# mgholamikn/PoseGen

Measured on AMD Instinct MI355X. Metric: rendered rays/sec (512x512, 64 samples/ray), higher is better.
Workload: dtype bf16

## Files before the change

posegen_amd/csrc/pg_device.h:

```cpp
#pragma once
#include <hip/hip_runtime.h>

#include <atomic>

#include "pg_program.h"

namespace pgd {
using namespace pgl;

typedef __attribute__((ext_vector_type(8))) __bf16 bf16x8;
typedef __attribute__((ext_vector_type(8))) _Float16 f16x8;
typedef __attribute__((ext_vector_type(16))) float f32x16;

struct EvalArgs {
    const float* rays;
    const float* z;
    const float* pts;
    const float* pnoise;
    const float* skts;
    const float* cams;
    const float* codes;
    const uint8_t* wstream;
    const uint8_t* wy;
    const float* rec_ab;
// ... 15 lines not shown
    int walk_rho;
};

struct RecArgs {
    const float* rays;
    const float* skts;
    const float* cams;
    const float* codes;
    const uint8_t* wy;
    float* rec_ab;
    uint8_t* rec_y;
    const float* z;
    long long pose_stride;
    int n_rays;
    int n_codes;
    int S;
};

struct PassWalk {
    int S, G, rho, pts;
    int dq[2], dr[2];
    int it, c;
    long long p0;
    int r0, off0;
    int itn, cn, r0n, off0n;
    long long p0n;
    static __host__ __device__ __forceinline__ int uni(int v) {
#if defined(__HIP_DEVICE_COMPILE__)
        return __builtin_amdgcn_readfirstlane(v);
#else
        return v;
#endif
    }
    __host__ __device__ __forceinline__ PassWalk(int S_, int pts_, int b, int G_, int rho_) : S(S_), G(G_), rho(rho_), pts(pts_) {
        const long long s0 = (long long)pts * (G + rho), s1 = (long long)pts * rho;
        dq[0] = uni((int)(s0 / S)); dr[0] = uni((int)(s0 % S));
        dq[1] = uni((int)(s1 / S)); dr[1] = uni((int)(s1 % S));
        it = c = b;
        p0 = (long long)b * pts;
        r0 = uni((int)(p0 / S));
        off0 = uni((int)(p0 - (long long)r0 * S));
        peek();
    }
    __host__ __device__ __forceinline__ void peek() {
        const int wrap = c + rho >= G ? 1 : 0;
        const int di = wrap ? rho : G + rho;
        itn = it + di;
        cn = c + rho - (wrap ? G : 0);
        p0n = p0 + (long long)di * pts;
        off0n = off0 + dr[wrap];
        r0n = r0 + dq[wrap];
        if (off0n >= S) { off0n -= S; ++r0n; }
    }
    __host__ __device__ __forceinline__ void advance() { it = itn; c = cn; p0 = p0n; r0 = r0n; off0 = off0n; }
};

template <const int (&P)[24]>
__device__ __forceinline__ int perm_dev(int s) {
    constexpr unsigned long long lo = [] { unsigned long long v = 0; for (int i = 0; i < 12; ++i) v |= (unsigned long long)P[i] << (5 * i); return v; }();
    constexpr unsigned long long hi = [] { unsigned long long v = 0; for (int i = 0; i < 12; ++i) v |= (unsigned long long)P[12 + i] << (5 * i); return v; }();
    return (int)(((s < 12 ? lo : hi) >> (5 * (s < 12 ? s : s - 12))) & 31);
}
__device__ __forceinline__ int slot_joint_dev(int s) { return perm_dev<PERM16>(s); }

inline hipError_t ensure_lds_attr(const void* fn, int bytes, std::atomic<unsigned long long>& done) {
    int dev = 0;
    hipError_t e = hipGetDevice(&dev);
    if (e != hipSuccess) return e;
    const unsigned long long bit = 1ull << (dev & 63);
    if (done.load(std::memory_order_acquire) & bit) return hipSuccess;
    e = hipFuncSetAttribute(fn, hipFuncAttributeMaxDynamicSharedMemorySize, bytes);
    if (e != hipSuccess) return e;
    done.fetch_or(bit, std::memory_order_release);
    return hipSuccess;
}

__device__ __forceinline__ void glds16(const void* g, void* l) {
    __builtin_amdgcn_global_load_lds((const __attribute__((address_space(1))) void*)g,
                                     (__attribute__((address_space(3))) void*)l, 16, 0, 0);
}

#ifndef PG_RING_SLOTS
#define PG_RING_SLOTS 3
#endif
#ifndef PG_DMA_BASE
#define PG_DMA_BASE 0
#endif
template <int NWAVE, int NCHUNK_, int NDMA = NWAVE, int MASK_NX = 0, int MASK_X0 = 0, int MASK_X1 = 0, int MASK_X2 = -1, bool AHEAD_ = false>
struct Stream {
    static constexpr bool AHEAD = AHEAD_;
    static constexpr int NSLOT = PG_RING_SLOTS;
    static constexpr int DEPTH = NSLOT - 1;
    static constexpr int PER = CHUNK_BYTES / 1024 / NDMA;
    const uint8_t* wstream;
    uint8_t* ring;
    int wave, lane;
    uint32_t next_off;
    uint32_t fill_slot;
    uint32_t rd_off;
    uint32_t ring_lds;
    uint32_t lane16;
    uint32_t pf_mask = 0u, nx_mask = 0u;

    __device__ __forceinline__ void skip_masked() {
        if constexpr (MASK_NX > 0) {
            const uint32_t c = next_off / CHUNK_BYTES;
            const uint32_t k0 = c - (uint32_t)MASK_X0, k1 = c - (uint32_t)MASK_X1, k2 = c - (uint32_t)MASK_X2;
            const uint32_t k = k0 < (uint32_t)MASK_NX ? k0 : (MASK_X2 >= 0 && k2 < (uint32_t)MASK_NX ? k2 : k1);
            if (k < (uint32_t)MASK_NX) next_off += (uint32_t)__builtin_ctz(~(pf_mask >> k)) * CHUNK_BYTES;
        }
    }
    __device__ __forceinline__ void advance() {
        next_off = next_off + CHUNK_BYTES == (uint32_t)NCHUNK_ * CHUNK_BYTES ? 0u : next_off + CHUNK_BYTES;
        if constexpr (MASK_NX > 0) {
            if (next_off == 0u) pf_mask = nx_mask;
            skip_masked();
        }
    }

    __device__ __forceinline__ bool dma_wave() const { return NDMA == NWAVE || (wave >= dma_base() && wave < dma_base() + NDMA); }
    static constexpr int dma_base() { return NDMA == NWAVE ? 0 : PG_DMA_BASE; }
    __device__ __forceinline__ void prefetch_next() {
        const uint8_t* src = wstream + next_off + ((wave - dma_base()) * (PER * 1024) + lane * 16);
        uint8_t* dst = ring + fill_slot * CHUNK_BYTES + (wave - dma_base()) * (PER * 1024);
        if (dma_wave()) {
#pragma unroll
            for (int i = 0; i < PER; ++i) glds16(src + i * 1024, dst + i * 1024);
        }
        advance();
        fill_slot = fill_slot + 1 == NSLOT ? 0u : fill_slot + 1;
        asm volatile("" : "+s"(next_off), "+s"(fill_slot));
    }
    __device__ __forceinline__ void start(uint32_t first_mask = 0u) {
        next_off = 0;
        fill_slot = 0;
        pf_mask = nx_mask = first_mask;
        skip_masked();
#pragma unroll
        for (int i = 0; i < DEPTH; ++i) prefetch_next();
        rd_off = (uint32_t)(NSLOT - 1) * CHUNK_BYTES + lane * 16;
    }
#if defined(PG_STAMPS)
    unsigned long long t_vm = 0, t_bar = 0;
    unsigned long long t_rel = 0, t_rst = 0, t_s0 = 0, t_s1 = 0;
    unsigned n_rst = 0;
    template <bool PRIMED = false>
    __device__ __forceinline__ void restart_stamp() {
        unsigned long long t;
        asm volatile("s_memtime %0\n\ts_waitcnt lgkmcnt(0)" : "=s"(t), "+s"(t_s0), "+s"(t_s1), "+s"(t_rel)::"memory");
        if (PRIMED) { t_vm += t_s1 - t_s0; t_bar += t_rel - t_s1; }
        t_rst += t - t_rel;
        n_rst += 1u;
    }
#endif
    __device__ __forceinline__ void enter(int ) {
#if defined(PG_STAMPS)
        unsigned long long s0, s1, s2;
        asm volatile("s_waitcnt lgkmcnt(0)\n\ts_memtime %0\n\ts_waitcnt lgkmcnt(0)" : "=s"(s0)::"memory");
        asm volatile("s_waitcnt vmcnt(%0)" ::"n"((DEPTH - 1) * PER) : "memory");
        asm volatile("s_memtime %0\n\ts_waitcnt lgkmcnt(0)" : "=s"(s1)::"memory");
        __builtin_amdgcn_s_barrier();
        asm volatile("s_memtime %0\n\ts_waitcnt lgkmcnt(0)" : "=s"(s2)::"memory");
        t_vm += s1 - s0;
        t_bar += s2 - s1;
#else
        asm volatile("s_waitcnt vmcnt(%0)" ::"n"((DEPTH - 1) * PER) : "memory");
        asm volatile("s_waitcnt lgkmcnt(0)" ::: "memory");
        __builtin_amdgcn_s_barrier();
#endif
        prefetch_next();
        rd_off = rd_off + CHUNK_BYTES >= (uint32_t)NSLOT * CHUNK_BYTES + lane * 16 ? rd_off - (NSLOT - 1) * CHUNK_BYTES
                                                                                  : rd_off + CHUNK_BYTES;
        asm volatile("" : "+v"(rd_off)::"memory");
    }
    uint32_t cur_src, cur_dst;
    static constexpr bool plain_ok(int c) {
        if (c < 0) return false;
        const int n = c + DEPTH + 1;
        if (n >= NCHUNK_) return false;
        if (MASK_NX > 0) {
            const int xs[3] = {MASK_X0, MASK_X1, MASK_X2};
            for (int i = 0; i < 3; ++i)
                if (xs[i] >= 0 && c + 1 <= xs[i] + MASK_NX - 1 && n >= xs[i]) return false;
        }
        return true;
    }
    static constexpr int WAIT_NEXT = 1, PRIMED = 2;
    __device__ __forceinline__ void wait_pieces(int fl) {
        if (AHEAD && (fl & WAIT_NEXT)) asm volatile("s_waitcnt vmcnt(0)" ::: "memory");
        else asm volatile("s_waitcnt vmcnt(%0)" ::"n"((DEPTH - 1) * PER) : "memory");
    }
    __device__ __forceinline__ void ring_step(bool plain) {
        cur_src = next_off + (wave - dma_base()) * (PER * 1024);
        cur_dst = fill_slot * CHUNK_BYTES + (wave - dma_base()) * (PER * 1024);
        if (plain) next_off += CHUNK_BYTES; else advance();
        fill_slot = fill_slot + 1 == NSLOT ? 0u : fill_slot + 1;
        asm volatile("" : "+s"(next_off), "+s"(fill_slot), "+s"(cur_src), "+s"(cur_dst));
        rd_off = rd_off + CHUNK_BYTES >= (uint32_t)NSLOT * CHUNK_BYTES + lane * 16 ? rd_off - (NSLOT - 1) * CHUNK_BYTES
                                                                                  : rd_off + CHUNK_BYTES;
        asm volatile("" : "+v"(rd_off)::"memory");
    }
    __device__ __forceinline__ void enter_split(bool plain = false, int fl = 0) {
        static_assert(!AHEAD || NDMA == NWAVE, "chunk entries of the A pipe that runs across them: every wave refills");
#if defined(PG_STAMPS)
        if (AHEAD && (fl & PRIMED)) {
            ring_step(plain);
            if (fl & WAIT_NEXT)
                asm volatile("s_memtime %0\n\ts_waitcnt vmcnt(0)\n\ts_memtime %1\n\ts_barrier\n\ts_memtime %2" : "=&s"(t_s0), "=&s"(t_s1), "=&s"(t_rel)::"memory");
            else
                asm volatile("s_memtime %0\n\ts_waitcnt vmcnt(%3)\n\ts_memtime %1\n\ts_barrier\n\ts_memtime %2" : "=&s"(t_s0), "=&s"(t_s1), "=&s"(t_rel) : "n"((DEPTH - 1) * PER) : "memory");
            return;
        }
        {
            unsigned long long s0, s1, s2;
            asm volatile("s_waitcnt lgkmcnt(0)\n\ts_memtime %0\n\ts_waitcnt lgkmcnt(0)" : "=s"(s0)::"memory");
            wait_pieces(fl);
            asm volatile("s_memtime %0\n\ts_waitcnt lgkmcnt(0)" : "=s"(s1)::"memory");
            __builtin_amdgcn_s_barrier();
            asm volatile("s_memtime %0\n\ts_waitcnt lgkmcnt(0)" : "=s"(s2)::"memory");
            t_vm += s1 - s0;
            t_bar += s2 - s1;
            t_rel = s2;
        }
#else
        if (dma_wave()) wait_pieces(fl);
        if (!(AHEAD && (fl & PRIMED))) asm volatile("s_waitcnt lgkmcnt(0)" ::: "memory");
#if !defined(PG_ABL_NOBARRIER)
        __builtin_amdgcn_s_barrier();
#endif
#endif
        ring_step(plain);
    }
    __device__ __forceinline__ void piece(int i) const {
#if defined(PG_ABL_NODMA)
        return;
#endif
        if (!dma_wave()) return;
#if defined(PG_VISIBLE_DMA)
        glds16(wstream + (cur_src + i * 1024) + lane16, ring + cur_dst + i * 1024);
        return;
#endif
        const uint8_t* sbase = wstream + (cur_src + i * 1024);
        asm volatile("s_mov_b32 m0, %0\n\ts_nop 0\n\tglobal_load_lds_dwordx4 %1, %2"
                     :: "s"(ring_lds + cur_dst + i * 1024), "v"(lane16), "s"(sbase) : "memory");
    }
    __device__ __forceinline__ const uint8_t* at(int , int byte_off) const {
        return ring + byte_off + rd_off;
    }
    template <typename R>
    __device__ __forceinline__ void issue(R& dst, int pos) const {
        const unsigned addr = ring_lds + rd_off;
        switch (pos) {
#define PG_ISSUE_CASE(P) case P: asm volatile("ds_read_b128 %0, %1 offset:" #P "*1024" : "=v"(dst) : "v"(addr)); break;
            PG_ISSUE_CASE(0) PG_ISSUE_CASE(1) PG_ISSUE_CASE(2) PG_ISSUE_CASE(3) PG_ISSUE_CASE(4) PG_ISSUE_CASE(5)
            PG_ISSUE_CASE(6) PG_ISSUE_CASE(7) PG_ISSUE_CASE(8) PG_ISSUE_CASE(9) PG_ISSUE_CASE(10) PG_ISSUE_CASE(11)
            PG_ISSUE_CASE(12) PG_ISSUE_CASE(13) PG_ISSUE_CASE(14) PG_ISSUE_CASE(15) PG_ISSUE_CASE(16) PG_ISSUE_CASE(17)
            PG_ISSUE_CASE(18) PG_ISSUE_CASE(19) PG_ISSUE_CASE(20) PG_ISSUE_CASE(21) PG_ISSUE_CASE(22) PG_ISSUE_CASE(23)
            PG_ISSUE_CASE(24) PG_ISSUE_CASE(25) PG_ISSUE_CASE(26) PG_ISSUE_CASE(27) PG_ISSUE_CASE(28) PG_ISSUE_CASE(29)
            PG_ISSUE_CASE(30) PG_ISSUE_CASE(31)
#undef PG_ISSUE_CASE
            default: __builtin_unreachable();
        }
    }
    template <typename R>
    __device__ __forceinline__ void issue_next(R& dst, int pos) const {
        const unsigned addr = ring_lds + rd_off + (fill_slot == (uint32_t)(NSLOT - 1) ? 0u - (uint32_t)((NSLOT - 1) * CHUNK_BYTES) : (uint32_t)CHUNK_BYTES);
        switch (pos) {
#define PG_ISSUE_CASE(P) case P: asm volatile("ds_read_b128 %0, %1 offset:" #P "*1024" : "=v"(dst) : "v"(addr)); break;
            PG_ISSUE_CASE(0) PG_ISSUE_CASE(1) PG_ISSUE_CASE(2) PG_ISSUE_CASE(3)
#undef PG_ISSUE_CASE
            default: __builtin_unreachable();
        }
    }
    __device__ __forceinline__ void drain() const { asm volatile("s_waitcnt vmcnt(0)" ::: "memory"); }
};

__device__ __forceinline__ f32x16 load_bias(const float* bias, int tile, int h) {
    const float4* p = reinterpret_cast<const float4*>(bias + (tile * 2 + h) * 16);
    const float4 a = p[0], b = p[1], c = p[2], d = p[3];
    f32x16 r = {a.x, a.y, a.z, a.w, b.x, b.y, b.z, b.w, c.x, c.y, c.z, c.w, d.x, d.y, d.z, d.w};
    return r;
}

__device__ __forceinline__ void lds_barrier() {
    asm volatile("s_waitcnt lgkmcnt(0)" ::: "memory");
    __builtin_amdgcn_s_barrier();
    asm volatile("" ::: "memory");
}

constexpr int LDS_RING = 0;
constexpr int LDS_BIAS = PG_RING_SLOTS * CHUNK_BYTES;
constexpr int LDS_CUT = LDS_BIAS + BIAS_FLOATS * 4;
constexpr int LDS_RTAB = LDS_CUT + 48 * 4;
constexpr int LDS_TOTAL = LDS_RTAB + MAXR * SLOT_FLOATS * 4;
static_assert(LDS_BIAS % 16 == 0 && LDS_CUT % 16 == 0 && LDS_RTAB % 16 == 0, "LDS alignment");
#if !defined(PG_RING_EXPERIMENT)
static_assert(LDS_TOTAL <= 160 * 1024, "LDS budget of one CU");
#endif

__device__ __forceinline__ void bone_local(const float* sk, float px, float py, float pz,
                                           float& qx, float& qy, float& qz) {
    const float4 a = *reinterpret_cast<const float4*>(sk);
    const float4 b = *reinterpret_cast<const float4*>(sk + 4);
    const float4 c = *reinterpret_cast<const float4*>(sk + 8);
    qx = fmaf(a.z, pz, fmaf(a.y, py, fmaf(a.x, px, a.w)));
    qy = fmaf(b.z, pz, fmaf(b.y, py, fmaf(b.x, px, b.w)));
// ... 155 lines not shown
```

posegen_amd/csrc/pg_eval16r.hip:

```cpp
#ifndef PG_PREFETCH
#define PG_PREFETCH 1
#endif
#ifndef PG_PIPE_H
#define PG_PIPE_H 4
#endif
#include <type_traits>

#include "pg_eval16_common.h"
#include "pg_launch.h"

#ifndef PG_REC_POLICY
#define PG_REC_POLICY ""
#endif

namespace pgd {

typedef __attribute__((ext_vector_type(4))) float f32x4;

template <typename V> struct Op16;
template <> struct Op16<bf16x8> {
    static __device__ __forceinline__ f32x4 mfma(bf16x8 a, bf16x8 b, f32x4 c) {
        return __builtin_amdgcn_mfma_f32_16x16x32_bf16(a, b, c, 0, 0, 0);
    }
};
// ... 106 lines not shown
    float f2[JG];
#pragma unroll
    for (int jj = 0; jj < JG; ++jj) { rp[jj][0].fetch(ab0, jj); rp[jj][1].fetch(ab1, jj); }
#pragma unroll
    for (int jj = 0; jj < JG; ++jj) f2[jj] = far2[jj];
    asm volatile("s_waitcnt lgkmcnt(0)" ::: "memory");
    int farmask = 0;
    float v[2][8];
#pragma unroll
    for (int jj = 0; jj < JG; ++jj) {
        float s2[2];
#pragma unroll
        for (int c = 0; c < 2; ++c) {
            float qx, qy, qz;
            rp[jj][c].q(c ? z1 : z0, qx, qy, qz);
            s2[c] = fmaf(qz, qz, fmaf(qx, qx, qy * qy));
            const float rinv = __builtin_amdgcn_rsqf(fmaxf(s2[c], 1e-24f));
            float* r3 = v[c] + 3 * (jj & 1);
            r3[0] = qx * rinv; r3[1] = qy * rinv; r3[2] = qz * rinv;
        }
        if (__builtin_amdgcn_ballot_w64(fminf(s2[0], s2[1]) < f2[jj]) == 0ull) farmask |= 1 << jj;
        if (jj & 1) {
#pragma unroll
            for (int c = 0; c < 2; ++c) {
                v[c][6] = v[c][7] = 0.0f;
                const u32x4 w = __builtin_bit_cast(u32x4, Op<V>::cvt(v[c]));
                unsigned w0 = w[0], w1 = w[1], w2 = w[2];
                asm volatile("" : "+v"(w0), "+v"(w1), "+v"(w2));
                const u32x4 o = {w0, w1, w2, 0u};
                xdir[jj / 2][c] = __builtin_bit_cast(V, o);
            }
        }
    }
    return farmask;
}

template <typename V>
__device__ __forceinline__ void y_code16(const float* yc, uint8_t* ylds, int nrm1, int tid) {
    using E = typename Op<V>::E;
    for (int idx = tid; idx < (nrm1 + 1) * VW; idx += NTHR) {
        const int ray = idx / VW, o = idx - ray * VW;
        *reinterpret_cast<E*>(ylds + ray * REC_Y_BYTES + (o >> 4) * 1024 + (o & 15) * 16 + 2 * JG) = (E)yc[idx];
    }
}

constexpr unsigned y_lane_tab(int i) {
    unsigned w = 0u;
    for (int g = 0; g < 4; ++g) {
        const int k = 8 * g + i, c = (k >= 9) + (k >= 18), r9 = k - 9 * c;
        const bool row = r9 >= 1 && k < 27;
        w |= (unsigned)(row ? (((r9 - 1) >> 1) << 1) | ((r9 - 1) & 1) : 0) << (8 * g);
    }
    return w;
}

template <typename V, typename ST>
__device__ __forceinline__ void y_segment16(ST& st, int gmask, const uint8_t* ab, uint8_t* ylds, int nrm1, int wave, int lane) {
    using E = typename Op<V>::E;
    constexpr int NQ = NTV16 / 2;
    if ((~gmask & ((1 << JG) - 1)) == 0) return;
    const int g = lane >> 4, col = lane & 15;
    const int gj = wave & 3, t0 = NQ * (wave >> 2);
    const uint8_t* row = ab + min(col, nrm1) * REC_AB_BYTES + (JG * gj) * 32 + 16;
    uint8_t* ydst = ylds + col * REC_Y_BYTES + t0 * 1024 + (gj * 16 + 4 * g) * 16;
    float fac[8], ph[8];
#pragma unroll
    for (int i = 0; i < 8; ++i) {
        const unsigned t = y_lane_tab(i) >> (8 * g);
        fac[i] = __builtin_bit_cast(float, 0x3f800000u + ((t & 6u) << 22));
        ph[i] = (t & 1u) ? 0.25f : 0.0f;
    }
    const bool g0 = g == 0, g1 = g == 1, g2 = g == 2, g3 = g == 3;
#pragma clang loop unroll(full)
    for (int jj = 0; jj < JG; ++jj) {
        if ((gmask >> jj) & 1) continue;
        st.enter_split();
#pragma unroll
        for (int i = 0; i < ST::PER; ++i) st.piece(i);
        const float4 b = *reinterpret_cast<const float4*>(row + jj * 32);
        V av[NQ];
#pragma unroll
        for (int q = 0; q < NQ; ++q)
            av[q] = __builtin_bit_cast(V, *reinterpret_cast<const uint4*>(st.at(0, (gj * NTV16 + t0 + q) * UNIT_BYTES)));
        __builtin_amdgcn_sched_barrier(0);
        const float inv = __builtin_amdgcn_rsqf(fmaxf(b.x * b.x + b.y * b.y + b.z * b.z, 1e-24f)) * 0.15915494309189535f;
        const float rx = b.x * inv, ry = b.y * inv, rz = b.z * inv;
        const float ehi = g0 ? rx : (g1 ? ry : rz), elo = g2 ? ry : (g3 ? rz : rx);
        float tv[8];
#pragma unroll
        for (int i = 0; i < 8; ++i) {
            const float ec = i == 0 ? elo : (i == 1 ? (g1 ? ehi : elo) : ehi);
            const float sv = __builtin_amdgcn_sinf(fmaf(ec, fac[i], ph[i]));
            const bool row0 = i == 0 ? g0 : (i == 1 ? g1 : (i == 2 && g2));
            tv[i] = (i >= 3 && g3) ? 0.0f : (row0 ? ec * 6.283185307179586f : sv);
        }
        const V bf = Op<V>::cvt(tv);
        f32x4 c4[NQ];
#pragma unroll
        for (int q = 0; q < NQ; ++q) c4[q] = Op16<V>::mfma(av[q], bf, f32x4{0.0f, 0.0f, 0.0f, 0.0f});
        if (col <= nrm1) {
#pragma unroll
            for (int q = 0; q < NQ; ++q) {
                E* dst = reinterpret_cast<E*>(ydst + q * 1024 + 2 * jj);
#pragma unroll
                for (int r = 0; r < 4; ++r) dst[r * 8] = (E)c4[q][r];
            }
        }
    }
}

__device__ __forceinline__ int pass_far_mask(const uint8_t* ab, int nrm1, const float* far2g, int g, int col) {
    const float* row = opaque_ptr(reinterpret_cast<const float*>(ab + min(col, nrm1) * REC_AB_BYTES) + JG * g * 8 + 3);
    int m = 0;
#pragma unroll
    for (int jj = 0; jj < JG; ++jj)
        if (__builtin_amdgcn_ballot_w64(row[jj * 8] < far2g[jj]) == 0ull) m |= 1 << jj;
    return __builtin_amdgcn_readfirstlane(m);
}

struct BiasPipe {
    unsigned base;
    a128 r;
    __device__ __forceinline__ BiasPipe(unsigned bbase, int tile0) { asm volatile("" : "+v"(bbase)); base = bbase + tile0 * 64; }
    __device__ __forceinline__ void fetch(int k) {
        switch (k) {
#define PG_BIAS_CASE(K) case K: asm volatile("ds_read_b128 %0, %1 offset:0+" #K "*64" : "=v"(r) : "v"(base)); break;
            PG_BIAS_CASE(0) PG_BIAS_CASE(1) PG_BIAS_CASE(2) PG_BIAS_CASE(3) PG_BIAS_CASE(4) PG_BIAS_CASE(5) PG_BIAS_CASE(6) PG_BIAS_CASE(7)
            PG_BIAS_CASE(8) PG_BIAS_CASE(9) PG_BIAS_CASE(10) PG_BIAS_CASE(11) PG_BIAS_CASE(12) PG_BIAS_CASE(13) PG_BIAS_CASE(14) PG_BIAS_CASE(15) PG_BIAS_CASE(16)
#undef PG_BIAS_CASE
            default: __builtin_unreachable();
        }
    }
    __device__ __forceinline__ void next_layer() { base += NT16 * 64; }
    __device__ __forceinline__ f32x4 take() { lds_landed(r); return __builtin_bit_cast(f32x4, r); }
};

template <typename V, int T, int NS, typename ST>
__device__ __forceinline__ void row_tile16(f32x4& acc0, f32x4& acc1, APipe<V, NS>& p, ST& st, int o, const V (*fin)[2]) {
#pragma unroll
    for (int u = 0; u < HU16; ++u) {
        const V av = next_a<V, T, true, NS>(p, st, o * HU16 + u);
        acc0 = Op16<V>::mfma(av, fin[u][0], acc0);
        acc1 = Op16<V>::mfma(av, fin[u][1], acc1);
    }
}

#ifndef PG_R_PACK_AT
#define PG_R_PACK_AT 2
#endif
#ifndef PG_R_BIAS_AT
#define PG_R_BIAS_AT 4
#endif
static_assert(PG_R_BIAS_AT <= HU16 - 3, "the bias fetch needs two more retires of the tile behind it");
template <typename V, int XM, int C0, typename ST>
__device__ __forceinline__ void hidden_layer16(const V (*fin)[2], V (*fout)[2], ST& st, APipe<V>& p, BiasPipe& bp) {
    constexpr int T = HU16 * NT16, c0 = C0;
    static_assert(!(ST::AHEAD && (XM & XM_IN_SEGMENT)) || (ST::plain_ok(C0) && ST::plain_ok(C0 + 1) && ST::plain_ok(C0 + 2) && ST::plain_ok(C0 + 3) && T == 4 * pgp::R::UPC),
                  "the entries of a layer whose pipe runs across them are straight-line");
    constexpr bool PRIMED = ST::AHEAD && (XM & XM_PRIMED) != 0, ON = ST::AHEAD && (XM & XM_HANDS_ON) != 0;
    f32x4 lo0, lo1, hi0, hi1;
    if ((XM & XM_PRIMED) != 0) bp.next_layer();
    if (!PRIMED) bp.fetch(0);
#pragma unroll
    for (int o = 0; o < NT16; ++o) {
        f32x4 acc0, acc1;
#pragma unroll
        for (int u = 0; u < HU16; ++u) {
            const V av = next_a<V, T, true, PG_PIPE_H, ST, XM>(p, st, o * HU16 + u, c0);
            if (u == 0) acc0 = acc1 = bp.take();
            acc0 = Op16<V>::mfma(av, fin[u][0], acc0);
            acc1 = Op16<V>::mfma(av, fin[u][1], acc1);
            if (u == PG_R_PACK_AT && o >= 2 && (o & 1) == 0) {
                if (PG_PIN_TILE) __builtin_amdgcn_sched_barrier(0);
                fout[o / 2 - 1][0] = relu_pack16<V>(lo0, hi0, true);
                fout[o / 2 - 1][1] = relu_pack16<V>(lo1, hi1, true);
                if (PG_PIN_TILE) __builtin_amdgcn_sched_barrier(0);
            }
            if (u == PG_R_BIAS_AT && (o + 1 < NT16 || ON)) bp.fetch(o + 1);
        }
        if (o & 1) { hi0 = acc0; hi1 = acc1; } else { lo0 = acc0; lo1 = acc1; }
    }
    fout[NT16 / 2 - 1][0] = relu_pack16<V>(lo0, hi0, true);
    fout[NT16 / 2 - 1][1] = relu_pack16<V>(lo1, hi1, true);
}

template <typename V, bool FC>
__device__ __forceinline__ void y_apply16(f32x4 (*vacc)[2], const uint8_t* ylds, const float (*wd)[JG],
                                          const int* myr, int lane) {
    const int g = lane >> 4;
    u32x4 w[2];
#pragma unroll
    for (int c = 0; c < 2; ++c) {
        float wx[8];
#pragma unroll
        for (int e = 0; e < JG; ++e) wx[e] = wd[c][e];
        wx[6] = (FC && g == 0) ? 1.0f : 0.0f;
        wx[7] = 0.0f;
        w[c] = __builtin_bit_cast(u32x4, Op<V>::cvt(wx));
    }
    const int ra = __builtin_amdgcn_readfirstlane(myr[0]);
    const int rb = __builtin_amdgcn_readlane(myr[1], 63);
    for (int ray = ra; ray <= rb; ++ray) {
        u32x4 b0, b1;
#pragma unroll
        for (int q = 0; q < 4; ++q) { b0[q] = myr[0] == ray ? w[0][q] : 0u; b1[q] = myr[1] == ray ? w[1][q] : 0u; }
        const uint8_t* yb = ylds + ray * REC_Y_BYTES + lane * 16;
#pragma unroll
        for (int t = 0; t < NTV16; ++t) {
            const V av = __builtin_bit_cast(V, *reinterpret_cast<const uint4*>(yb + t * 1024));
            vacc[t][0] = Op16<V>::mfma(av, __builtin_bit_cast(V, b0), vacc[t][0]);
            vacc[t][1] = Op16<V>::mfma(av, __builtin_bit_cast(V, b1), vacc[t][1]);
        }
    }
}

template <typename V, bool FC, bool TAPS, bool OC, bool CNT = false, bool PP = false>
__global__ __launch_bounds__(NTHR, 2) void eval16r_kernel(const EvalArgs a) {
    static_assert(!PP || OC, "per-ray poses without records are a form of the on-chip variant");
    extern __shared__ __attribute__((aligned(16))) uint8_t smem[];
    float* bias = reinterpret_cast<float*>(smem + LDSR_BIAS);
    float* cut = reinterpret_cast<float*>(smem + LDSR_CUT);
    const int tid = threadIdx.x, lane = tid & 63, wave = __builtin_amdgcn_readfirstlane(tid >> 6);
    const int g = lane >> 4, col = lane & 15;
    const uint32_t lds0 = (uint32_t)(uintptr_t)(__attribute__((address_space(3))) uint8_t*)smem;
    const uint32_t lane16 = (uint32_t)lane * 16u;
    using ST = typename std::conditional<OC, StreamRO, StreamR>::type;
    ST st{a.wstream, smem + LDSR_RING, wave, lane, 0u, 0u, 0u, lds0 + LDSR_RING, lane16};
    const uint8_t* rec_ab = reinterpret_cast<const uint8_t*>(a.rec_ab);
    const float* sk_lds = reinterpret_cast<const float*>(smem + LDSR_SK);
    const float* stage = reinterpret_cast<const float*>(smem + LDSR_STAGE);

    for (int i = tid; i < BIAS16_FLOATS; i += NTHR) bias[i] = a.bias[i];
    auto uniform = [](float x) { float s; asm volatile("s_nop 0\n\tv_readfirstlane_b32 %0, %1\n\ts_nop 1" : "=s"(s) : "v"(x)); return s; };
    const float tlv = uniform(a.tau_v * 1.4426950408889634f), tld = uniform(a.tau_d * 1.4426950408889634f);
    if (tid < 48) cut[tid] = -a.cutoff[(tid < J ? 0 : J) + slot_joint_dev(tid < J ? tid : tid - J)] * (tid < J ? tlv : tld);
    else if (tid < 72) {
        const int jt = slot_joint_dev(tid - 48);
        const float far = fmaxf(tlv > 0.0f ? a.cutoff[jt] + 24.0f / tlv : __builtin_inff(), tld > 0.0f ? a.cutoff[J + jt] + 24.0f / tld : __builtin_inff());
        cut[tid] = far * far;
    }
    if (OC) {
        if (!PP) for (int i = tid; i < J * 12; i += NTHR) reinterpret_cast<float*>(smem + LDSR_SK)[i] = a.skts[slot_joint_dev(i / 12) * 16 + i % 12];
        for (int i = tid; i < MAXR_F * REC_Y_BYTES / 16; i += NTHR) reinterpret_cast<uint4*>(smem + LDSR_Y)[i] = make_uint4(0u, 0u, 0u, 0u);
    }
#if defined(PG_YOUNG_PRIO)
    if (wave >= NWAVE / 2) __builtin_amdgcn_s_setprio(PG_YOUNG_PRIO);
#endif
    const unsigned bbase = lds_addr_of(bias) + 16 * g;
    PassWalk pw(a.S, PTS, (int)blockIdx.x, (int)gridDim.x, a.walk_rho);
    long long p0 = pw.p0;
    int r0 = pw.r0, off0 = pw.off0;
    if (OC) {
        lds_barrier();
        if (tid < MAXR_F * J) {
            const int k = tid / J, sl = tid - k * J;
            const long long ray = min((long long)r0 + k, (long long)a.n_rays - 1);
            const float* skr = PP ? a.skts + ray * a.pose_stride + slot_joint_dev(sl) * 16 : sk_lds + sl * 12;
            ab_row(skr, a.rays + ray * 11, a.z[ray * a.S], a.z[ray * a.S + a.S - 1],
                   reinterpret_cast<float4*>(smem + LDSR_AB + k * REC_AB_BYTES + sl * 32));
        }
    } else if ((int)blockIdx.x < a.n_iters && wave < LDS_AB_BYTES / 1024)
        dma_piece(rec_ab + (long long)r0 * REC_AB_BYTES + wave * 1024, lds0 + LDSR_AB + wave * 1024, lane16);
    if (OC && FC) {
        const float* ytab = reinterpret_cast<const float*>(a.wy);
        for (int idx = tid; idx < MAXR_F * VW; idx += NTHR) {
            const int k = idx / VW, o = idx - k * VW;
            const float cf = a.cams ? a.cams[min((long long)r0 + k, (long long)a.n_rays - 1)] : -1.0f;
            const int ci = cf < 0.0f ? a.n_codes : min((int)cf, a.n_codes - 1);
            reinterpret_cast<float*>(smem + LDSR_YC)[idx] = ytab[(long long)ci * VW + o];
        }
    }
    asm volatile("s_waitcnt vmcnt(0)" ::: "memory");
    lds_barrier();
    int abuf = 0;
    auto rays_of_pass = [&](long long p0_, int off0_) {
        const int last_ = (int)max(0ll, min((long long)PTS - 1, a.n_points - 1 - p0_));
        const int t_ = off0_ + last_;
        return (t_ >= a.S) + (t_ >= 2 * a.S) + (t_ >= 3 * a.S) + (t_ >= 4 * a.S);
    };
    int gmask = 0;
#if !defined(PG_NO_FAR_SKIP)
    gmask = pass_far_mask(smem + LDSR_AB, rays_of_pass(p0, off0), cut + 2 * J + JG * g, g, col);
    if (!a.far_skip) gmask = 0;
#endif
    st.start((uint32_t)gmask);

    float nx_z[2] = {0.0f, 0.0f};
#define PG_PREFETCH_Z(itn, col_)                                                                   \
    do {                                                                                           \
        const long long p0n_ = (long long)(itn) * PTS + wave * 32 + (col_);                        \
        nx_z[0] = a.z[min(p0n_, a.n_points - 1)];                                                  \
        nx_z[1] = a.z[min(p0n_ + 16, a.n_points - 1)];                                             \
    } while (0)
    if ((int)blockIdx.x < a.n_iters) PG_PREFETCH_Z(blockIdx.x, col);

#if defined(PG_STAMPS)
    unsigned long long stamps[16];
#define PG_XSTAMPS(k) (stamps + (k))
    unsigned long long rst_t[2];
    unsigned rst_n[2];
#define PG_RST_OPEN(k) do { rst_t[k] = st.t_rst; rst_n[k] = st.n_rst; } while (0)
#define PG_RST_CLOSE(k) do { rst_t[k] = st.t_rst - rst_t[k]; rst_n[k] = st.n_rst - rst_n[k]; } while (0)
#else
#define PG_XSTAMPS(k) nullptr
#define PG_RST_OPEN(k) do {} while (0)
#define PG_RST_CLOSE(k) do {} while (0)
#endif
#if defined(PG_WALK_STAMPS)
    unsigned long long walk_t0;
    asm volatile("s_memtime %0\n\ts_waitcnt lgkmcnt(0)" : "=s"(walk_t0) :: "memory");
    unsigned walk_passes = 0, walk_limbs = 0;
#endif
    for (int it = pw.it; it < a.n_iters; it = pw.it) {
        PG_STAMP(0);
        int lane_p = lane;
        asm volatile("" : "+v"(lane_p));
        const int g_p = lane_p >> 4;
        const int last = (int)min((long long)PTS - 1, a.n_points - 1 - p0);
        const int S1 = a.S, S2 = 2 * a.S, S3 = 3 * a.S, S4 = 4 * a.S;
        auto ray_of = [&](int t) { return (t >= S1) + (t >= S2) + (t >= S3) + (t >= S4); };
        const int nrm1 = ray_of(off0 + last);
        int myr[2];
        float zz[2];
        const float* abp[2];
#pragma unroll
        for (int c = 0; c < 2; ++c) {
            const int i = wave * 32 + 16 * c + (lane_p & 15);
            myr[c] = min(ray_of(off0 + i), nrm1);
            zz[c] = nx_z[c];
            abp[c] = opaque_ptr(reinterpret_cast<const float*>(smem + LDSR_AB + abuf * LDS_AB_BYTES + myr[c] * REC_AB_BYTES) + JG * g_p * 8);
        }
        const int itn = min(pw.itn, a.n_iters - 1);
        const int off0n = pw.off0n, r0n = pw.r0n;
        const float* cutd = opaque_ptr(cut + J + JG * g_p);
        const QFromAB q0{abp[0], zz[0]}, q1{abp[1], zz[1]};
        const float* cutv = opaque_ptr(cut + JG * g_p);
        V xdir[JG / 2][2];
        int farmask = dir_operands16<V>(xdir, lds_addr_of(abp[0]), lds_addr_of(abp[1]), zz[0], zz[1], opaque_ptr(cut + 2 * J + JG * g_p));
#if defined(PG_NO_FAR_SKIP)
        farmask = 0;
#else
        farmask = __builtin_amdgcn_readfirstlane(a.far_skip ? farmask : 0);
#endif
#if defined(PG_WALK_STAMPS)
        walk_passes += 1; walk_limbs += (unsigned)__builtin_popcount(~gmask & 63);
#endif
        if (CNT && lane == 0) {
            if (wave == 0) { atomicAdd(reinterpret_cast<unsigned*>(a.dbg), 1u); atomicAdd(reinterpret_cast<unsigned*>(a.dbg) + 1, (unsigned)__builtin_popcount(gmask)); }
            atomicAdd(reinterpret_cast<unsigned*>(a.dbg) + 2, (unsigned)__builtin_popcount(farmask));
        }
        auto fetch_records = [&]() {
            if (OC) {
                const long long rn = min((long long)r0n, (long long)a.n_rays - 1);
                if (wave == 0) dma_dwords(a.rays, (uint32_t)(min(rn * 11 + lane_p, (long long)a.n_rays * 11 - 1) * 4), lds0 + LDSR_STAGE);
                else if (wave == 1) {
                    const long long ray = min(rn + min(lane_p >> 1, MAXR_F - 1), (long long)a.n_rays - 1);
                    dma_dwords(a.z, (uint32_t)((ray * a.S + ((lane_p & 1) ? a.S - 1 : 0)) * 4), lds0 + LDSR_STAGE + 256);
                } else if (FC && wave == 2 && a.cams)
                    dma_dwords(a.cams, (uint32_t)(min(rn + min(lane_p, MAXR_F - 1), (long long)a.n_rays - 1) * 4), lds0 + LDSR_STAGE + 512);
                return;
            }
            const uint8_t* ysrc = a.rec_y + (size_t)r0 * REC_Y_BYTES + wave * 1024;
#pragma unroll
            for (int k = 0; k < MAXR_F; ++k)
                dma_piece(ysrc + (size_t)min(k, nrm1) * REC_Y_BYTES, lds0 + LDSR_Y + k * REC_Y_BYTES + wave * 1024, lane16);
            if (wave < LDS_AB_BYTES / 1024)
                dma_piece(rec_ab + (long long)min(r0n, a.n_rays - 1) * REC_AB_BYTES + wave * 1024,
                          lds0 + LDSR_AB + (abuf ^ 1) * LDS_AB_BYTES + wave * 1024, lane16);
        };

        PG_STAMP(1);
        constexpr int CH = pgp::R::CH_HID;
        constexpr int C_L1 = pgp::R::CH_L0X + (OC ? pgp::R::NLIMB : 0), C_L5H = C_L1 + 4 * CH, C_L6 = C_L5H + CH + pgp::R::CH_L0X, C_AV = C_L6 + 2 * CH;
        static_assert(C_L5H + CH == (OC ? pgp::R::C_L5X_OC : pgp::R::C_L5X) && C_AV + pgp::R::CH_AVR == (OC ? pgp::R::NCHUNK_OC : pgp::R::NCHUNK),
                      "chunk bases follow pg_program.h");
        V fa[HU16][2], fb[HU16][2];
        {
            f32x4 acc[NT16][2];
#pragma unroll
            for (int o = 0; o < NT16; ++o) acc[o][0] = acc[o][1] = load_bias16(bias, BS_LAYER0 + o, g);
            x_segment16<V>(acc, st, abp[0], abp[1], zz[0], zz[1], cutv, tlv, farmask, gmask, xdir, fetch_records, PG_XSTAMPS(12));
            if (TAPS && a.dbg && a.dbg_stage == 0) {
#pragma unroll
                for (int c = 0; c < 2; ++c) {
                    const int i = wave * 32 + 16 * c + (lane_p & 15);
                    if (i <= last) {
#pragma unroll
                        for (int o = 0; o < NT16; ++o)
#pragma unroll
                            for (int r = 0; r < 4; ++r) a.dbg[(p0 + i) * W + 16 * o + 4 * g_p + r] = acc[o][c][r];
                    }
                }
            }
#pragma unroll
            for (int u = 0; u < HU16; ++u)
#pragma unroll
                for (int c = 0; c < 2; ++c) fa[u][c] = relu_pack16<V>(acc[2 * u][c], acc[2 * u + 1][c], true);
        }
        PG_STAMP(11);
        if constexpr (OC) {
            y_segment16<V>(st, gmask, smem + LDSR_AB + abuf * LDS_AB_BYTES, smem + LDSR_Y, nrm1, wave, lane_p);
            if (FC) y_code16<V>(reinterpret_cast<const float*>(smem + LDSR_YC + abuf * LDSR_YC_BYTES), smem + LDSR_Y, nrm1, wave * 64 + lane_p);
        }
        PG_STAMP(2);
        PG_RST_OPEN(0);
        constexpr int XM_H = XM_IN_SEGMENT;
        APipe<V> ph;
        BiasPipe bp1(bbase, BS_LAYER0 + 1 * NT16);
        hidden_layer16<V, XM_H, C_L1>(fa, fb, st, ph, bp1);
        if constexpr (OC) {
            if (FC && wave < MAXR_F) {
                const float cf = a.cams ? stage[128 + wave] : -1.0f;
                const int ci = __builtin_amdgcn_readfirstlane(cf < 0.0f ? a.n_codes : min((int)cf, a.n_codes - 1));
                const uint32_t dst = lds0 + LDSR_YC + (abuf ^ 1) * LDSR_YC_BYTES + wave * (VW * 4);
                dma_dwords(a.wy, (uint32_t)((ci * VW + lane_p) * 4), dst);
                dma_dwords(a.wy, (uint32_t)((ci * VW + 64 + lane_p) * 4), dst + 256);
            }
            const int item = wave * 15 + (lane_p & 15);
            if (lane_p < 15) {
                const int k = item / J, sl = item - k * J;
                const float* skr = PP ? a.skts + min((long long)r0n + k, (long long)a.n_rays - 1) * a.pose_stride + slot_joint_dev(sl) * 16 : sk_lds + sl * 12;
                ab_row(skr, stage + 11 * k, stage[64 + 2 * k], stage[64 + 2 * k + 1],
                       reinterpret_cast<float4*>(smem + LDSR_AB + (abuf ^ 1) * LDS_AB_BYTES + k * REC_AB_BYTES + sl * 32));
            }
        }
        BiasPipe bp2(bbase, BS_LAYER0 + 2 * NT16);
        hidden_layer16<V, XM_H | XM_HANDS_ON, C_L1 + CH>(fb, fa, st, ph, bp2);
        hidden_layer16<V, XM_H | XM_PRIMED | XM_HANDS_ON, C_L1 + 2 * CH>(fa, fb, st, ph, bp2);
        hidden_layer16<V, XM_H | XM_PRIMED, C_L1 + 3 * CH>(fb, fa, st, ph, bp2);
        PG_RST_CLOSE(0);
        PG_STAMP(3);
        {
            f32x4 acc[NT16][2];
            APipeX<V> p5;
            BiasPipe bp(bbase, BS_LAYER0 + 5 * NT16);
            bp.fetch(0);
#pragma unroll
            for (int o = 0; o < NT16; ++o) {
#pragma unroll
                for (int u = 0; u < HU16; ++u) {
                    const V av = next_a<V, HU16 * NT16, true, PG_PIPE_X>(p5, st, o * HU16 + u, C_L5H);
                    if (u == 0) acc[o][0] = acc[o][1] = bp.take();
                    acc[o][0] = Op16<V>::mfma(av, fa[u][0], acc[o][0]);
                    acc[o][1] = Op16<V>::mfma(av, fa[u][1], acc[o][1]);
                    if (u == PG_R_BIAS_AT && o + 1 < NT16) bp.fetch(o + 1);
                }
            }
            x_segment16<V>(acc, st, abp[0], abp[1], zz[0], zz[1], cutv, tlv, farmask, gmask, xdir, [] {}, PG_XSTAMPS(14));
#pragma unroll
            for (int u = 0; u < HU16; ++u)
#pragma unroll
                for (int c = 0; c < 2; ++c) fb[u][c] = relu_pack16<V>(acc[2 * u][c], acc[2 * u + 1][c], true);
        }
        PG_STAMP(4);
        PG_RST_OPEN(1);
        BiasPipe bp6(bbase, BS_LAYER0 + 6 * NT16);
        hidden_layer16<V, XM_H | XM_HANDS_ON, C_L6>(fb, fa, st, ph, bp6);
        hidden_layer16<V, XM_H | XM_PRIMED, C_L6 + CH>(fa, fb, st, ph, bp6);
        PG_RST_CLOSE(1);
        PG_STAMP(5);
        int gmask_n = 0;
#if !defined(PG_NO_FAR_SKIP)
        gmask_n = pass_far_mask(smem + LDSR_AB + (abuf ^ 1) * LDS_AB_BYTES, rays_of_pass(pw.p0n, off0n),
                                opaque_ptr(cut + 2 * J + JG * g_p), g_p, lane_p & 15);
        if (!a.far_skip) gmask_n = 0;
#endif
        st.nx_mask = (uint32_t)gmask_n;
        float sigma[2];
        f32x4 c0, c1;
        {
            APipe<V> pv;
            constexpr int TAV = pgp::R::U_AV;
            static_assert(BS_VIEWF == BS_ALPHA + 1 && BS_RGB == BS_VIEWF + NTV16, "alpha, view and rgb bias tiles are consecutive");
            BiasPipe bp(bbase, BS_ALPHA);
            bp.fetch(0);
            auto av_tile = [&](int o, f32x4& t0, f32x4& t1) __attribute__((always_inline)) {
#pragma unroll
                for (int u = 0; u < HU16; ++u) {
                    const V av = next_a<V, TAV, true, PG_PIPE_H>(pv, st, o * HU16 + u, C_AV);
                    if (u == 0) t0 = t1 = bp.take();
                    t0 = Op16<V>::mfma(av, fb[u][0], t0);
                    t1 = Op16<V>::mfma(av, fb[u][1], t1);
                    if (u == PG_R_BIAS_AT && o < NTV16) bp.fetch(o + 1);
                }
            };
            {
                f32x4 t0, t1;
                av_tile(0, t0, t1);
                sigma[0] = t0[0]; sigma[1] = t1[0];
            }
            bool empty = false;
            if (CNT || a.skip_empty) {
                const int i = wave * 32 + (lane_p & 15);
                const bool live = g_p == 0 && ((i <= last && !(sigma[0] <= 0.0f)) || (i + 16 <= last && !(sigma[1] <= 0.0f)));
                empty = __builtin_amdgcn_ballot_w64(live) == 0ull;
                if (CNT && lane == 0 && empty) {
                    atomicAdd(reinterpret_cast<unsigned*>(a.dbg) + 3, 1u);
                    if (a.skip_empty) atomicAdd(reinterpret_cast<unsigned*>(a.dbg) + 4, 1u);
                }
                empty = empty && a.skip_empty != 0;
            }
            if (empty) {
                asm volatile("s_waitcnt lgkmcnt(0)" ::: "memory");
                PG_STAMP(6);
                skip_units<TAV, HU16>(st, C_AV);
                PG_STAMP(7);
                PG_PREFETCH_Z(itn, lane_p & 15);
                c0 = c1 = f32x4{0.0f, 0.0f, 0.0f, 0.0f};
            } else {
                f32x4 vacc[NTV16][2];
                V fg[NTV16 / 2][2];
#pragma unroll
                for (int o = 1; o < NTV16 + 1; ++o) av_tile(o, vacc[o - 1][0], vacc[o - 1][1]);
                PG_STAMP(6);
                float wd[2][JG];
#pragma unroll
                for (int jj = 0; jj < JG; ++jj) {
                    float qx, qy, qz;
                    q0(jj, qx, qy, qz);
                    wd[0][jj] = cutoff_weight_fast(__builtin_amdgcn_sqrtf(qx * qx + qy * qy + qz * qz), tld, cutd[jj]);
                    q1(jj, qx, qy, qz);
                    wd[1][jj] = cutoff_weight_fast(__builtin_amdgcn_sqrtf(qx * qx + qy * qy + qz * qz), tld, cutd[jj]);
                    if (OC && ((gmask >> jj) & 1)) wd[0][jj] = wd[1][jj] = 0.0f;
                }
                y_apply16<V, FC>(vacc, smem + LDSR_Y, wd, myr, lane_p);
#pragma unroll
                for (int u = 0; u < NTV16 / 2; ++u)
#pragma unroll
                    for (int c = 0; c < 2; ++c) fg[u][c] = relu_pack16<V>(vacc[2 * u][c], vacc[2 * u + 1][c], true);
                PG_STAMP(7);
                PG_PREFETCH_Z(itn, lane_p & 15);
                APipe<V> pr;
                BiasPipe bpr(bbase, BS_RGB);
                bpr.fetch(0);
#pragma unroll
                for (int u = 0; u < pgp::R::U_RGB; ++u) {
                    const V av = next_a_cont<V, pgp::R::U_RGB, PG_PIPE_H, pgp::R::U_AV % UPC>(pr, st, u);
                    if (u == 0) c0 = c1 = bpr.take();
                    c0 = Op16<V>::mfma(av, fg[u][0], c0);
                    c1 = Op16<V>::mfma(av, fg[u][1], c1);
                }
            }
        }
        if (g_p == 0) {
            const int i = wave * 32 + (lane_p & 15);
            if (i <= last) *reinterpret_cast<float4*>(a.raw + (p0 + i) * 4) = make_float4(c0[0], c0[1], c0[2], sigma[0]);
            if (i + 16 <= last) *reinterpret_cast<float4*>(a.raw + (p0 + i + 16) * 4) = make_float4(c1[0], c1[1], c1[2], sigma[1]);
        }
        abuf ^= 1;
        pw.advance(); pw.peek();
        p0 = pw.p0; r0 = pw.r0; off0 = pw.off0;
        gmask = gmask_n;
        PG_STAMP(8);
#if defined(PG_STAMPS)
        {
            const int every = max(1, a.n_iters / 1024), slot = it / every;
            if (a.dbg && a.dbg_stage == 99 && lane == 0 && slot * every == it && slot < 1024) {
                unsigned long long* rec = reinterpret_cast<unsigned long long*>(a.dbg) + ((long long)slot * NWAVE + wave) * 24;
                for (int k = 0; k < 9; ++k) rec[k] = stamps[k];
                rec[9] = st.t_vm; rec[10] = st.t_bar;
                rec[11] = stamps[11];
                for (int k = 12; k < 16; ++k) rec[k] = stamps[k];
                rec[16] = st.t_rst; rec[17] = st.n_rst;
                rec[18] = rst_t[0]; rec[19] = rst_n[0];
                rec[20] = rst_t[1]; rec[21] = rst_n[1];
                rec[22] = rec[23] = 0;
            }
            st.t_vm = 0; st.t_bar = 0; st.t_rst = 0; st.n_rst = 0u;
        }
#endif
    }
    st.drain();
#if defined(PG_WALK_STAMPS)
    if (CNT && tid == 0) {
        unsigned long long walk_t1;
        asm volatile("s_memtime %0\n\ts_waitcnt lgkmcnt(0)" : "=s"(walk_t1) :: "memory");
        unsigned* rec = reinterpret_cast<unsigned*>(a.dbg) + 16 + 8 * blockIdx.x;
        rec[0] = (unsigned)walk_t0; rec[1] = (unsigned)(walk_t0 >> 32);
        rec[2] = (unsigned)walk_t1; rec[3] = (unsigned)(walk_t1 >> 32);
        rec[4] = walk_passes; rec[5] = walk_limbs;
    }
#endif
}

template <typename V, bool FC, bool TAPS, bool OC, bool CNT = false, bool PP = false>
static hipError_t launch_eval16r(const EvalArgs& a, int grid, hipStream_t stream) {
    auto k = eval16r_kernel<V, FC, TAPS, OC, CNT, PP>;
    constexpr int lds = OC ? LDSR_TOTAL_OC : LDSR_TOTAL;
    static std::atomic<unsigned long long> attr_done{0};
    const hipError_t ae = ensure_lds_attr(reinterpret_cast<const void*>(k), lds, attr_done);
    if (ae != hipSuccess) return ae;
    hipLaunchKernelGGL(k, dim3(grid), dim3(NTHR), lds, stream, a);
    return hipGetLastError();
}

template <typename V>
static hipError_t dispatch_eval16r(const EvalArgs& a, int framecode, int onchip, int grid, hipStream_t s) {
    if (onchip) {
        if (a.dbg && a.dbg_stage != 99 && a.dbg_stage != 97) return hipErrorInvalidValue;
        const bool pp = a.pose_stride != 0;
        if (a.dbg && a.dbg_stage == 97) return (pp || framecode) ? hipErrorInvalidValue : launch_eval16r<V, false, false, true, true>(a, grid, s);
        if (framecode) return pp ? launch_eval16r<V, true, false, true, false, true>(a, grid, s) : launch_eval16r<V, true, false, true>(a, grid, s);
        return pp ? launch_eval16r<V, false, false, true, false, true>(a, grid, s) : launch_eval16r<V, false, false, true>(a, grid, s);
    }
    const bool taps = a.dbg && a.dbg_stage != 99;
    if (taps) return framecode ? launch_eval16r<V, true, true, false>(a, grid, s) : launch_eval16r<V, false, true, false>(a, grid, s);
    return framecode ? launch_eval16r<V, true, false, false>(a, grid, s) : launch_eval16r<V, false, false, false>(a, grid, s);
}

}

extern "C" int pg_launch_eval16r(const pgd::EvalArgs* a, int fp16, int framecode, int onchip, int grid, void* stream) {
    using namespace pgd;
    hipStream_t s = static_cast<hipStream_t>(stream);
    if (onchip && framecode && !a->wy) return (int)hipErrorInvalidValue;
    return (int)(fp16 ? dispatch_eval16r<f16x8>(*a, framecode, onchip, grid, s) : dispatch_eval16r<bf16x8>(*a, framecode, onchip, grid, s));
}
```

Baseline: 9.076 million.

## Spread ReLU-pack of hidden activations across MFMA slots and carry across layers

Replaces the bursty relu_pack16 of each tile pair with a PackJob that interleaves per-element cvt_pk and pk_max_i16 steps between the MFMAs of the following tiles. The last tile pair of a layer marked hands-on is carried into the next layer and finished inside that layer's first tile, instead of being packed at the layer boundary. The aim is to hide the conversion VALU work under MFMA latency and shorten the gap between layers. It adds inline asm that the compiler cannot reschedule, so the interleaving is only as good as the chosen step slots. Optional stamp instrumentation and asm markers are also added for profiling.

```diff
diff --git a/posegen_amd/csrc/pg_device.h b/posegen_amd/csrc/pg_device.h
--- a/posegen_amd/csrc/pg_device.h
+++ b/posegen_amd/csrc/pg_device.h
@@ -191,6 +191,15 @@
         t_rst += t - t_rel;
         n_rst += 1u;
     }
+    unsigned long long t_pk0 = 0, t_pk = 0;
+    unsigned n_pk = 0;
+    __device__ __forceinline__ void pack_stamp_open() { asm volatile("s_memtime %0" : "=s"(t_pk0)::"memory"); }
+    __device__ __forceinline__ void pack_stamp_close() {
+        unsigned long long t;
+        asm volatile("s_memtime %0\n\ts_waitcnt lgkmcnt(0)" : "=s"(t), "+s"(t_pk0)::"memory");
+        t_pk += t - t_pk0;
+        n_pk += 1u;
+    }
 #endif
     __device__ __forceinline__ void enter(int ) {
 #if defined(PG_STAMPS)
diff --git a/posegen_amd/csrc/pg_eval16r.hip b/posegen_amd/csrc/pg_eval16r.hip
--- a/posegen_amd/csrc/pg_eval16r.hip
+++ b/posegen_amd/csrc/pg_eval16r.hip
@@ -282,25 +282,97 @@
 #define PG_R_BIAS_AT 4
 #endif
 static_assert(PG_R_BIAS_AT <= HU16 - 3, "the bias fetch needs two more retires of the tile behind it");
+template <typename V> struct CvtPk;
+template <> struct CvtPk<bf16x8> {
+    static __device__ __forceinline__ unsigned one(float x, float y) { unsigned d; asm volatile("v_cvt_pk_bf16_f32 %0, %1, %2" : "=v"(d) : "v"(x), "v"(y)); return d; }
+};
+template <> struct CvtPk<f16x8> {
+    static __device__ __forceinline__ unsigned one(float x, float y) { unsigned d; asm volatile("v_cvt_pk_f16_f32 %0, %1, %2" : "=v"(d) : "v"(x), "v"(y)); return d; }
+};
+
+template <typename V> struct PackJob {
+    f32x4 acc[2][2];
+    unsigned w[2][4];
+    __device__ __forceinline__ void step(int k, V (*fout)[2], int slot) {
+#if defined(PG_ABL_NOPACK)
+        if (k == 11 || k == 15) fout[slot][(k - 8) >> 2] = __builtin_bit_cast(V, acc[0][(k - 8) >> 2]);
+        return;
+#endif
+        if (k < 8) {
+            const int h = k >> 2, c = (k >> 1) & 1, half = k & 1;
+            w[c][2 * h + half] = CvtPk<V>::one(acc[h][c][2 * half], acc[h][c][2 * half + 1]);
+        } else {
+            const int c = (k - 8) >> 2, d = (k - 8) & 3;
+            unsigned r;
+            asm volatile("v_pk_max_i16 %0, %1, 0" : "=v"(r) : "v"(w[c][d]));
+            w[c][d] = r;
+            if (d == 3) {
+                const u32x4 o = {w[c][0], w[c][1], w[c][2], w[c][3]};
+                fout[slot][c] = __builtin_bit_cast(V, o);
+            }
+        }
+    }
+};
+__device__ __forceinline__ constexpr int carry_lo_step(int u) { return u <= 4 ? u - 1 : (u <= 6 ? 8 + (u - 5) : 12); }
+constexpr int CARRY_LO_LAST = 13;
+constexpr int CARRY_U0 = 2, CARRY_U1 = 5;
+__device__ __forceinline__ constexpr int carry_hi_step(int u, int i) { return u - CARRY_U0 < 2 ? 4 + 2 * (u - CARRY_U0) + i : (u - CARRY_U0 == 2 ? 10 + i : 14 + i); }
+static_assert(CARRY_U0 >= 2 && CARRY_U1 - CARRY_U0 == 3 && CARRY_U1 + 2 <= HU16 - 1,
+              "the carried pair: the younger tile's last MFMA is at least two MFMAs old, and the MFMAs of a whole unit lie in front of the fragment's first use");
+
 template <typename V, int XM, int C0, typename ST>
-__device__ __forceinline__ void hidden_layer16(const V (*fin)[2], V (*fout)[2], ST& st, APipe<V>& p, BiasPipe& bp) {
+__device__ __forceinline__ void hidden_layer16(V (*fin)[2], V (*fout)[2], ST& st, APipe<V>& p, BiasPipe& bp, PackJob<V>& carry) {
     constexpr int T = HU16 * NT16, c0 = C0;
     static_assert(!(ST::AHEAD && (XM & XM_IN_SEGMENT)) || (ST::plain_ok(C0) && ST::plain_ok(C0 + 1) && ST::plain_ok(C0 + 2) && ST::plain_ok(C0 + 3) && T == 4 * pgp::R::UPC),
                   "the entries of a layer whose pipe runs across them are straight-line");
     constexpr bool PRIMED = ST::AHEAD && (XM & XM_PRIMED) != 0, ON = ST::AHEAD && (XM & XM_HANDS_ON) != 0;
+#if defined(PG_PACK_BURST)
+    constexpr bool SPREAD = false;
+#else
+    constexpr bool SPREAD = true;
+#endif
+    constexpr bool CARRY_IN = SPREAD && (XM & XM_PRIMED) != 0, CARRY_OUT = SPREAD && (XM & XM_HANDS_ON) != 0;
     f32x4 lo0, lo1, hi0, hi1;
+    PackJob<V> job;
     if ((XM & XM_PRIMED) != 0) bp.next_layer();
     if (!PRIMED) bp.fetch(0);
 #pragma unroll
     for (int o = 0; o < NT16; ++o) {
         f32x4 acc0, acc1;
+        if (o == (CARRY_IN ? 0 : 1)) asm volatile("; PG_HIDDEN begin");
+        if (SPREAD && o >= 2 && (o & 1) == 0) { job.acc[0][0] = lo0; job.acc[0][1] = lo1; job.acc[1][0] = hi0; job.acc[1][1] = hi1; }
 #pragma unroll
         for (int u = 0; u < HU16; ++u) {
+            const int q = (o * HU16 + u) % pgp::R::UPC;
+            const bool entry = q == 0 || q >= pgp::R::UPC - (PG_PIPE_H - 1);
+            if (entry) asm volatile("; PG_ENTRY begin");
             const V av = next_a<V, T, true, PG_PIPE_H, ST, XM>(p, st, o * HU16 + u, c0);
+            if (entry) asm volatile("; PG_ENTRY end");
             if (u == 0) acc0 = acc1 = bp.take();
+#if defined(PG_STAMPS)
+            if (u == PG_R_PACK_AT + 1 && o >= 2 && (o & 1) == 0) st.pack_stamp_close();
+#endif
+            if (SPREAD) {
+                const bool any = o >= 2 || (CARRY_IN && o == 0 && u >= CARRY_U0 - 1 && u <= CARRY_U1);
+                if (any && PG_PIN_TILE) __builtin_amdgcn_sched_barrier(0);
+                if (o >= 2) { job.step((o & 1) * HU16 + u, fout, o / 2 - 1); }
+                if (CARRY_OUT && o == NT16 - 1) {
+                    if (u == 0) { carry.acc[0][0] = lo0; carry.acc[0][1] = lo1; }
+                    else carry.step(carry_lo_step(u), fout, NT16 / 2 - 1);
+                }
+                if (CARRY_IN && o == 0 && u == CARRY_U0 - 1) carry.step(CARRY_LO_LAST, fin, NT16 / 2 - 1);
+                if (CARRY_IN && o == 0 && u >= CARRY_U0 && u <= CARRY_U1) {
+                    carry.step(carry_hi_step(u, 0), fin, NT16 / 2 - 1);
+                    carry.step(carry_hi_step(u, 1), fin, NT16 / 2 - 1);
+                }
+                if (any && PG_PIN_TILE) __builtin_amdgcn_sched_barrier(0);
+            }
             acc0 = Op16<V>::mfma(av, fin[u][0], acc0);
             acc1 = Op16<V>::mfma(av, fin[u][1], acc1);
-            if (u == PG_R_PACK_AT && o >= 2 && (o & 1) == 0) {
+#if defined(PG_STAMPS)
+            if (u == PG_R_PACK_AT && o >= 2 && (o & 1) == 0) { __builtin_amdgcn_sched_barrier(0); st.pack_stamp_open(); }
+#endif
+            if (!SPREAD && u == PG_R_PACK_AT && o >= 2 && (o & 1) == 0) {
                 if (PG_PIN_TILE) __builtin_amdgcn_sched_barrier(0);
                 fout[o / 2 - 1][0] = relu_pack16<V>(lo0, hi0, true);
                 fout[o / 2 - 1][1] = relu_pack16<V>(lo1, hi1, true);
@@ -310,8 +382,16 @@
         }
         if (o & 1) { hi0 = acc0; hi1 = acc1; } else { lo0 = acc0; lo1 = acc1; }
     }
+    if (SPREAD && PG_PIN_TILE) __builtin_amdgcn_sched_barrier(0);
+    asm volatile("; PG_HIDDEN end");
+    if (CARRY_OUT) {
+        carry.acc[1][0] = hi0; carry.acc[1][1] = hi1;
+        return;
+    }
+    asm volatile("; PG_PACKBLOCK begin");
     fout[NT16 / 2 - 1][0] = relu_pack16<V>(lo0, hi0, true);
     fout[NT16 / 2 - 1][1] = relu_pack16<V>(lo1, hi1, true);
+    asm volatile("; PG_PACKBLOCK end");
 }
 
 template <typename V, bool FC>
@@ -429,8 +509,10 @@
 #define PG_XSTAMPS(k) (stamps + (k))
     unsigned long long rst_t[2];
     unsigned rst_n[2];
-#define PG_RST_OPEN(k) do { rst_t[k] = st.t_rst; rst_n[k] = st.n_rst; } while (0)
-#define PG_RST_CLOSE(k) do { rst_t[k] = st.t_rst - rst_t[k]; rst_n[k] = st.n_rst - rst_n[k]; } while (0)
+    unsigned long long pk_t[2];
+    unsigned pk_n[2];
+#define PG_RST_OPEN(k) do { rst_t[k] = st.t_rst; rst_n[k] = st.n_rst; pk_t[k] = st.t_pk; pk_n[k] = st.n_pk; } while (0)
+#define PG_RST_CLOSE(k) do { rst_t[k] = st.t_rst - rst_t[k]; rst_n[k] = st.n_rst - rst_n[k]; pk_t[k] = st.t_pk - pk_t[k]; pk_n[k] = st.n_pk - pk_n[k]; } while (0)
 #else
 #define PG_XSTAMPS(k) nullptr
 #define PG_RST_OPEN(k) do {} while (0)
@@ -536,8 +618,9 @@
         PG_RST_OPEN(0);
         constexpr int XM_H = XM_IN_SEGMENT;
         APipe<V> ph;
+        PackJob<V> pj;
         BiasPipe bp1(bbase, BS_LAYER0 + 1 * NT16);
-        hidden_layer16<V, XM_H, C_L1>(fa, fb, st, ph, bp1);
+        hidden_layer16<V, XM_H, C_L1>(fa, fb, st, ph, bp1, pj);
         if constexpr (OC) {
             if (FC && wave < MAXR_F) {
                 const float cf = a.cams ? stage[128 + wave] : -1.0f;
@@ -555,9 +638,9 @@
             }
         }
         BiasPipe bp2(bbase, BS_LAYER0 + 2 * NT16);
-        hidden_layer16<V, XM_H | XM_HANDS_ON, C_L1 + CH>(fb, fa, st, ph, bp2);
-        hidden_layer16<V, XM_H | XM_PRIMED | XM_HANDS_ON, C_L1 + 2 * CH>(fa, fb, st, ph, bp2);
-        hidden_layer16<V, XM_H | XM_PRIMED, C_L1 + 3 * CH>(fb, fa, st, ph, bp2);
+        hidden_layer16<V, XM_H | XM_HANDS_ON, C_L1 + CH>(fb, fa, st, ph, bp2, pj);
+        hidden_layer16<V, XM_H | XM_PRIMED | XM_HANDS_ON, C_L1 + 2 * CH>(fa, fb, st, ph, bp2, pj);
+        hidden_layer16<V, XM_H | XM_PRIMED, C_L1 + 3 * CH>(fb, fa, st, ph, bp2, pj);
         PG_RST_CLOSE(0);
         PG_STAMP(3);
         {
@@ -585,8 +668,8 @@
         PG_STAMP(4);
         PG_RST_OPEN(1);
         BiasPipe bp6(bbase, BS_LAYER0 + 6 * NT16);
-        hidden_layer16<V, XM_H | XM_HANDS_ON, C_L6>(fb, fa, st, ph, bp6);
-        hidden_layer16<V, XM_H | XM_PRIMED, C_L6 + CH>(fa, fb, st, ph, bp6);
+        hidden_layer16<V, XM_H | XM_HANDS_ON, C_L6>(fb, fa, st, ph, bp6, pj);
+        hidden_layer16<V, XM_H | XM_PRIMED, C_L6 + CH>(fa, fb, st, ph, bp6, pj);
         PG_RST_CLOSE(1);
         PG_STAMP(5);
         int gmask_n = 0;
@@ -694,9 +777,10 @@
                 rec[16] = st.t_rst; rec[17] = st.n_rst;
                 rec[18] = rst_t[0]; rec[19] = rst_n[0];
                 rec[20] = rst_t[1]; rec[21] = rst_n[1];
-                rec[22] = rec[23] = 0;
-            }
-            st.t_vm = 0; st.t_bar = 0; st.t_rst = 0; st.n_rst = 0u;
+                rec[22] = (pk_t[0] & 0xffffffffull) | (pk_t[1] << 32);
+                rec[23] = (unsigned long long)pk_n[0] | ((unsigned long long)pk_n[1] << 32);
+            }
+            st.t_vm = 0; st.t_bar = 0; st.t_rst = 0; st.n_rst = 0u; st.t_pk = 0; st.n_pk = 0u;
         }
 #endif
     }
```

Result: no change. 9.107 million, median of 3 (+0.3%).
